# sevagh/xumx-sliCQ

Hardware: AMD Instinct MI355X
Metric: real-time factor (audio-s demixed / wall-s), 44.1 kHz stereo, offline model (higher is better)
Workload: dtype f32; 1 GPU; BASELINE configs[1]: offline model (Bark-262 sliCQT), one 240 s stereo track (10,584,000 samples, 5 chunks) per GPU, Wiener off (mix-phase), seeded synthetic weights; parallelism=one track per rank, 1 rank(s), no data-path collective

## Files before the change

### xumx_slicq_amd/csrc/plan.h

```cpp
#pragma once
#include <algorithm>
#include <map>
#include <mutex>
#include <tuple>
#include <vector>

#include <rocfft/rocfft.h>

#include "common.h"

namespace xsq {

struct FftPlan {
    rocfft_plan plan = nullptr;
    rocfft_execution_info info = nullptr;
    size_t work_bytes = 0;
};

struct TileTable {
    TileDev* d_tiles = nullptr;
    int ntiles = 0;
};

enum class TileKind { BandGemm, Dft4Full, CdaeGemm, CdaeSlab, CdaeWino, CdaeL1f, CdaeL4f };
struct TileKey {
    TileKind kind;
    int rows, S;
    int sub, flags;
    bool operator<(const TileKey& o) const {
        return std::tie(kind, rows, S, sub, flags) < std::tie(o.kind, o.rows, o.S, o.sub, o.flags);
    }
};

template <class D, class T>
static int upload(D*& dst, const T* src, size_t count) {
    dst = nullptr;
    if (!count) return XSQ_OK;
    XSQ_HIP(hipMalloc((void**)&dst, count * sizeof(T)));
    const hipError_t e = hipMemcpy(dst, src, count * sizeof(T), hipMemcpyHostToDevice);
    if (e != hipSuccess) { (void)hipFree(dst); dst = nullptr; }
    XSQ_HIP(e);
    return XSQ_OK;
}
template <class D, class T>
static int upload(D*& dst, const std::vector<T>& vec) { return upload(dst, vec.data(), vec.size()); }

template <class T, class Fill>
static int cached_tiles(std::mutex& mu, std::map<TileKey, TileTable>& cache, const TileKey& key, TileTable* out, Fill&& fill) {
    std::lock_guard<std::mutex> lk(mu);
    auto it = cache.find(key);
    if (it != cache.end()) { *out = it->second; return XSQ_OK; }
    std::vector<T> t;
    fill(t);
    TileTable tt;
    tt.ntiles = (int)t.size();
    if (int rc = upload(tt.d_tiles, t)) return rc;
    cache[key] = tt;
    *out = tt;
    return XSQ_OK;
}

template <class KeyFn>
static std::vector<int> order_descending(int n, KeyFn key) {
    std::vector<int> order(n);
    for (int i = 0; i < n; ++i) order[i] = i;
    std::stable_sort(order.begin(), order.end(), [&](int x, int y) { return key(x) > key(y); });
    return order;
}

struct BlockHost {
    int first_band, F, T;
    int64_t cum;
};

}

struct xsq_plan {
    int L = 0, tr = 0, h = 0, nbins = 0, nbands = 0, nblocks = 0;
    int64_t sumFT = 0;
    std::vector<xsq::BandDev> bands;
    std::vector<xsq::BlockHost> blocks;
    int band_radix4 = 1;
    void* d_bands4 = nullptr;
    float* d_pool4f = nullptr;
    float* d_pool4i = nullptr;
    int nbands4 = 0;
    std::vector<unsigned char> bands4_host;
    int64_t d4_max_block = 0;
    std::vector<int> bands4_m, bands4_small;
    int fft_backend = 0;
    float2* d_T = nullptr;
    unsigned short* d_tgt16 = nullptr;
    int* d_tgt = nullptr;
    int phase_begin[5] = {0, 0, 0, 0, 0};
    int packed_fft = 0;
    int short_inline = 0;
    void *d_s_item1 = nullptr, *d_s_tw1 = nullptr;
    int *d_s_item2 = nullptr, *d_s_tgt = nullptr;
    float* d_s_wd = nullptr;
    int short_n1 = 0, short_n2 = 0, short_nent = 0, short_sc0 = 0;
    int short_begin[5] = {0, 0, 0, 0, 0};
    int phase_long[4] = {0, 0, 0, 0};
    float* d_tw = nullptr;
    float* d_Wf = nullptr;
    float* d_Wi = nullptr;
    xsq::BandDev* d_bands = nullptr;
    int* d_cov_ptr = nullptr;
    int* d_cov_band = nullptr;
    std::mutex mu;
    std::map<std::pair<int, int>, xsq::FftPlan> fft;
    std::map<xsq::TileKey, xsq::TileTable> tiles;
};
```

### xumx_slicq_amd/csrc/slicqt.hip

```cpp
#include <algorithm>
#include <cmath>
#include <cstdarg>
#include <cstdio>
#include <cstdlib>
#include <cstring>

#include "../../include/xumx_slicq_hip.h"
#include "gemm_tile.h"
#include "plan.h"
#include "prof.h"
#include "slice_fft.h"
#include "band_dft4.h"
#include "band_dft4s.h"

namespace xsq {

static thread_local char g_err[1024] = "";
void set_error(const char* fmt, ...) {
    va_list ap;
    va_start(ap, fmt);
    vsnprintf(g_err, sizeof(g_err), fmt, ap);
    va_end(ap);
}

__global__ __launch_bounds__(256) void k_slice_window(const float* __restrict__ x,
                                                       const float* __restrict__ tw,
                                                       float* __restrict__ seg, int S, int64_t n, int L,
                                                       int h, const int64_t* __restrict__ xrows = nullptr,
                                                       const float* const* __restrict__ xslot = nullptr) {
    const int p = blockIdx.x * 256 + threadIdx.x;
    if (p >= L) return;
    const int row = blockIdx.y;
    const int bc = row / S, s = row - bc * S;
    const int64_t i = (int64_t)(2 * s - 2) * h + p;
    float v = 0.f;
    if (i >= 0 && i < n) v = tw[p] * (xslot ? *xslot : x)[(xrows ? xrows[bc] : (int64_t)bc * n) + i];
    seg[(int64_t)row * L + p] = v;
}

__global__ __launch_bounds__(256) void k_spectrum_gather(const float* __restrict__ Z,
                                                          const BandDev* __restrict__ bands,
                                                          const int* __restrict__ cov_ptr,
                                                          const int* __restrict__ cov_band,
                                                          float2* __restrict__ fr, int BC, int S, int nbins) {
    const int k = blockIdx.x * 256 + threadIdx.x;
    if (k >= nbins) return;
    const int row = blockIdx.y;
    const int bc = row / S, s = row - bc * S;
    const int64_t BCS = (int64_t)BC * S;
    float2 acc = make_float2(0.f, 0.f);
    for (int e = cov_ptr[k]; e < cov_ptr[k + 1]; ++e) {
        const BandDev b = bands[cov_band[e]];
        const int64_t off = 2 * (BCS * b.cum + (((int64_t)bc * b.F + b.f) * S + s) * b.Lg + (k - b.bin0));
        const float2 z = *reinterpret_cast<const float2*>(Z + off);
        acc.x += z.x;
        acc.y += z.y;
    }
    if (k == 0 || k == nbins - 1) acc.y = 0.f;
    fr[(int64_t)row * nbins + k] = acc;
}

__global__ __launch_bounds__(256) void k_overlap_add(const float* __restrict__ seg, float* __restrict__ y,
                                                      const int64_t* __restrict__ row_off,
                                                      int S, int64_t length, int L, int h) {
    const int64_t i = (int64_t)blockIdx.x * 256 + threadIdx.x;
    if (i >= length) return;
// ... 130 lines not shown
        if (mask) { v.x *= mk.x; v.y *= mk.x; v.z *= mk.y; v.w *= mk.y; }
        return v;
    }
    __device__ void epilogue(const Group& g, int row0, int n, const f32x16& a0, const f32x16& a1, bool wide) const {
        const bool c0 = n < g.N, c1 = wide && n + 32 < g.N;
#pragma unroll
        for (int r = 0; r < 16; ++r) {
            const int m = row0 + acc_row(r);
            if (m >= g.M) break;
            float* d = (row_len ? Z + 2 * ((int64_t)m * row_len + g.bin0) : Z + row_off(g, m)) + n;
            if (c0) d[0] = a0[r];
            if (c1) d[32] = a1[r];
        }
    }
};

constexpr int REMIX_MAX_BLOCKS = 256;
struct RemixArgs {
    const float* src;
    float* dst;
    int nch, R, S, cplx;
    float g[4][4];
    int use[4];
    int cum[REMIX_MAX_BLOCKS + 1];
};

__global__ __launch_bounds__(256) void k_remix_combine(RemixArgs a) {
#pragma clang fp contract(off)
    const int j = blockIdx.y, ch = blockIdx.z;
    const int64_t per = (int64_t)a.S * (a.cum[j + 1] - a.cum[j]) * a.cplx;
    const int64_t e = ((int64_t)blockIdx.x * 256 + threadIdx.x) * 4;
    if (e >= per) return;
    const int64_t base = (int64_t)a.S * a.cum[j] * a.cplx;
    const float* s = a.src + base * (4 * a.nch) + (int64_t)ch * per + e;
    float4 m[4];
#pragma unroll
    for (int t = 0; t < 4; ++t)
        m[t] = a.use[t] ? *reinterpret_cast<const float4*>(s + (int64_t)t * a.nch * per) : make_float4(0.f, 0.f, 0.f, 0.f);
    float* d = a.dst + base * ((int64_t)a.R * a.nch) + (int64_t)ch * per + e;
#pragma unroll
    for (int r = 0; r < 4; ++r) {
        if (r >= a.R) break;
        float4 acc = make_float4(0.f, 0.f, 0.f, 0.f);
#pragma unroll
        for (int t = 0; t < 4; ++t) {
            if (!a.use[t]) continue;
            const float g = a.g[r][t];
            acc.x = acc.x + g * m[t].x; acc.y = acc.y + g * m[t].y; acc.z = acc.z + g * m[t].z; acc.w = acc.w + g * m[t].w;
        }
        *reinterpret_cast<float4*>(d + (int64_t)r * a.nch * per) = acc;
    }
}

static int get_band_tiles(xsq_plan* P, int rows, TileTable* out) {
    const bool r4 = P->band_radix4 && P->nbands4 > 0;
    return cached_tiles<TileDev>(P->mu, P->tiles, TileKey{TileKind::BandGemm, rows, 0, 0, r4 ? 1 : 0}, out, [&](std::vector<TileDev>& t) {
        if (r4) {
            for (int i = (int)P->bands4_small.size() - 1; i >= 0; --i)
                push_group_tiles(t, P->bands4_small[i], rows, 2 * P->bands[P->bands4_small[i]].Lg);
        } else {
            for (int j = P->nbands - 1; j >= 0; --j) push_group_tiles(t, j, rows, 2 * P->bands[j].Lg);
        }
    });
}

#ifndef XSQ_D4_MIN_LG_DEFAULT
#define XSQ_D4_MIN_LG_DEFAULT 24
#endif

struct Switches {
    bool d4_sym = true;
    int d4_min_lg = XSQ_D4_MIN_LG_DEFAULT;
    Switches() {
        if (const char* e = getenv("XSQ_D4_SYM")) d4_sym = atoi(e) != 0;
        if (const char* e = getenv("XSQ_D4_MIN_LG")) d4_min_lg = atoi(e) >= 16 ? atoi(e) : d4_min_lg;
    }
};
static const Switches& switches() { static const Switches sw; return sw; }

static int get_dft4_full_tiles(xsq_plan* P, int rows, TileTable* out, int share, bool sym) {
    return cached_tiles<Tile4Dev>(P->mu, P->tiles, TileKey{TileKind::Dft4Full, rows, share, 0, sym ? 1 : 0}, out, [&](std::vector<Tile4Dev>& t) {
        const Band4Dev* b4 = reinterpret_cast<const Band4Dev*>(P->bands4_host.data());
        const int span = share > 0 ? share : rows, copies = share > 0 ? rows / share : 1;
        for (int i = P->nbands4 - 1; i >= 0; --i) {
            int ncb = (2 * P->bands4_m[i] + 15) / 16;
            if (sym) ncb = (P->bands4_m[i] / 2 + 1 + 15) / 16;
            for (int m0 = 0; m0 < span; m0 += D4H_ROWS)
                for (int k = 0; k < copies; ++k) t.push_back(Tile4Dev{m0 + k * span, ncb, b4[i]});
        }
    });
}

static int d4_ranges_ok(const xsq_plan* P, int64_t rows, const char* who) {
    if (!(P->band_radix4 && P->nbands4)) return XSQ_OK;
    XSQ_REQUIRE(8 * rows * P->d4_max_block < (1ll << 30) && (int64_t)8 * D4H_ROWS * std::max<int64_t>(P->nbins, P->sumFT) < (1ll << 30),
                "%s: %lld rows x %lld coefficients of a band block exceed 2^30 bytes; split the call (fewer stacked chunks)",
                who, (long long)rows, (long long)P->d4_max_block);
    return XSQ_OK;
}

template <bool FWD>
static int launch_dft4(xsq_plan* P, const Band4Args& a4, int rows, int share, hipStream_t stream) {
    const bool sym = switches().d4_sym;
    const bool masked = !FWD && a4.mask != nullptr;
    TileTable t;
    if (int rc = get_dft4_full_tiles(P, rows, &t, share, sym)) return rc;
    if (!t.ntiles) return XSQ_OK;
    auto kernel = masked ? band_dft4s_kernel<false, true> : band_dft4s_kernel<FWD, false>;
    if (!sym) kernel = masked ? band_dft4_full_kernel<false, 10, true> : band_dft4_full_kernel<FWD, 10, false>;
    hipLaunchKernelGGL(kernel, dim3(t.ntiles), dim3(sym ? 256 : D4H_NT), 0, stream, a4, (const Tile4Dev*)t.d_tiles, t.ntiles);
    return XSQ_OK;
}

static int get_fft(xsq_plan* P, int inverse, int batch, FftPlan* out) {
    std::lock_guard<std::mutex> lk(P->mu);
    auto key = std::make_pair(inverse, batch);
    auto it = P->fft.find(key);
    if (it != P->fft.end()) {
        *out = it->second;
        return XSQ_OK;
    }
    static std::once_flag once;
    std::call_once(once, [] { rocfft_setup(); });
    FftPlan f;
    size_t len = (size_t)P->L;
    rocfft_status st = rocfft_plan_create(&f.plan, rocfft_placement_notinplace,
                                          inverse ? rocfft_transform_type_real_inverse
                                                  : rocfft_transform_type_real_forward,
                                          rocfft_precision_single, 1, &len, (size_t)batch, nullptr);
    if (st != rocfft_status_success) {
        set_error("rocfft_plan_create(L=%d, batch=%d, inverse=%d) failed: %d", P->L, batch, inverse, (int)st);
        return XSQ_ERR_FFT;
    }
    rocfft_plan_get_work_buffer_size(f.plan, &f.work_bytes);
    if (rocfft_execution_info_create(&f.info) != rocfft_status_success) {
        set_error("rocfft_execution_info_create failed");
        return XSQ_ERR_FFT;
    }
    P->fft[key] = f;
    *out = f;
    return XSQ_OK;
}

static int run_fft(const FftPlan& f, void* in, void* out, void* work, hipStream_t stream) {
    if (rocfft_execution_info_set_stream(f.info, stream) != rocfft_status_success) {
        set_error("rocfft_execution_info_set_stream failed");
        return XSQ_ERR_FFT;
    }
    if (f.work_bytes) {
        if (rocfft_execution_info_set_work_buffer(f.info, work, f.work_bytes) != rocfft_status_success) {
            set_error("rocfft_execution_info_set_work_buffer failed");
            return XSQ_ERR_FFT;
        }
    }
    void* ib[1] = {in};
    void* ob[1] = {out};
    rocfft_status st = rocfft_execute(f.plan, ib, ob, f.info);
    if (st != rocfft_status_success) {
        set_error("rocfft_execute failed: %d", (int)st);
        return XSQ_ERR_FFT;
    }
    return XSQ_OK;
}
// ... 88 lines not shown
        }
    }
}

static void build_coverage(const xsq_plan* P, std::vector<int>& cov_ptr, std::vector<int>& cov_band) {
    cov_ptr.assign(P->nbins + 1, 0);
    std::vector<std::vector<int>> cov(P->nbins);
    for (int j = 0; j < P->nbands; ++j)
        for (int p = 0; p < P->bands[j].Lg; ++p) {
            const int k = P->bands[j].bin0 + p;
            if (k >= 0 && k <= P->L / 2) cov[k].push_back(j);
        }
    for (int k = 0; k < P->nbins; ++k) {
        cov_ptr[k + 1] = cov_ptr[k] + (int)cov[k].size();
        cov_band.insert(cov_band.end(), cov[k].begin(), cov[k].end());
    }
}

static bool build_slice_fft_tables(xsq_plan* P, std::vector<float2>& T, std::vector<int>& tgt, std::vector<unsigned short>& tgt16) {
    const int L = P->L, nbands = P->nbands;
    auto W = [&](int64_t j) {
        j %= L;
        return make_float2((float)std::cos(PI2 * j / L), (float)(-std::sin(PI2 * j / L)));
    };
    for (int k1 = 0; k1 < FFT_R1; ++k1)
        for (int m = 0; m < FFT_M1; ++m) T.push_back(W(2 * (int64_t)k1 * m));
    for (int k2 = 0; k2 < FFT_R2; ++k2)
        for (int n3 = 0; n3 < FFT_R3; ++n3) T.push_back(W(2 * (int64_t)FFT_R1 * n3 * k2));
    for (int k = 0; k <= FFT_N; ++k) T.push_back(W(k));
    bool ok = true;
    for (int ph = 0; ph < 4; ++ph) {
        P->phase_begin[ph] = (int)tgt.size();
        int last_end = -(1 << 30);
        for (int j = ph; j < nbands; j += 4) {
            BandDev& b = P->bands[j];
            b.ent = (int)tgt.size();
            const int lo = b.bin0 < 0 ? 0 : b.bin0;
            if (lo < last_end) ok = false;
            last_end = b.bin0 + b.Lg > L / 2 + 1 ? L / 2 + 1 : b.bin0 + b.Lg;
            for (int q = 0; q < b.Lg; ++q) {
                const int k = b.bin0 + q;
                tgt.push_back(k >= 0 && k <= L / 2 ? k : -1);
            }
        }
    }
    P->phase_begin[4] = (int)tgt.size();
    tgt16.assign(tgt.size() + 2, 0xFFFFu);
    for (size_t i = 0; i < tgt.size(); ++i) tgt16[i] = tgt[i] >= 0 ? (unsigned short)tgt[i] : 0xFFFFu;
    return ok;
}

static void build_radix4_tables(xsq_plan* P, const PlanArgs& A, std::vector<Band4Dev>& b4, std::vector<float>& pf, std::vector<float>& pi,
                                std::vector<char>& is_short) {
    const int d4_min_lg = switches().d4_min_lg;
    is_short.assign(A.nbands, 0);
    std::map<int, int64_t> doff, twoff, coff;
    auto alloc2 = [&](size_t n) { size_t o = pf.size(); pf.resize(o + n, 0.f); pi.resize(o + n, 0.f); return (int64_t)o; };
    for (int j = 0; j < A.nbands; ++j) {
        const BandDev& b = P->bands[j];
        if (b.Lg < d4_min_lg || b.Lg > 4 * D4_MPAD) { P->bands4_small.push_back(j); is_short[j] = 1; continue; }
        const int n = b.Lg, m = n / 4;
        Band4Dev d;
        memset(&d, 0, sizeof(d));
        d.Lg = n; d.m = m; d.bin0 = b.bin0; d.f = b.f; d.F = b.F; d.ent = b.ent; d.cum = b.cum; d.jband = j;
        d.ldd = (int)round_up(2 * m, 16);
        if (!doff.count(m)) {
            const int64_t o = alloc2((size_t)round_up(2 * m, 64) * d.ldd);
            doff[m] = o;
            for (int k = 0; k < m; ++k)
                for (int t1 = 0; t1 < m; ++t1) {
                    const int r = (int)(((int64_t)k * t1) % m);
                    const double cr = std::cos(PI2 * r / m), si = std::sin(PI2 * r / m);
                    for (int dir = 0; dir < 2; ++dir) {
                        std::vector<float>& pool = dir ? pi : pf;
                        const double dre = cr, dim = dir ? -si : si;
                        pool[o + (size_t)(2 * k) * d.ldd + 2 * t1] = (float)dre;
                        pool[o + (size_t)(2 * k) * d.ldd + 2 * t1 + 1] = (float)(-dim);
                        pool[o + (size_t)(2 * k + 1) * d.ldd + 2 * t1] = (float)dim;
                        pool[o + (size_t)(2 * k + 1) * d.ldd + 2 * t1 + 1] = (float)dre;
                    }
                }
        }
        d.d_off = doff[m];
        d.K2 = m / 2 + 1; d.ldc = (int)round_up(d.K2, 8);
        if (!coff.count(m)) {
            const size_t csz = (size_t)round_up(d.K2, 16) * d.ldc;
            const int64_t o = alloc2(2 * csz);
            coff[m] = o;
            for (int k = 0; k < d.K2; ++k)
                for (int nn = 0; nn < d.K2; ++nn) {
                    const int r = (int)(((int64_t)k * nn) % m);
                    const double cr = std::cos(PI2 * r / m), si = (nn == 0 || 2 * nn == m) ? 0.0 : std::sin(PI2 * r / m);
                    pf[o + (size_t)k * d.ldc + nn] = (float)cr;
                    pi[o + (size_t)k * d.ldc + nn] = (float)cr;
                    pf[o + csz + (size_t)k * d.ldc + nn] = (float)(-si);
                    pi[o + csz + (size_t)k * d.ldc + nn] = (float)si;
                }
        }
        d.c_off = coff[m];
        if (!twoff.count(n)) {
            const int mpad = (m + 7) & ~7;
            const int64_t o = alloc2((size_t)3 * mpad * 2);
            twoff[n] = o;
            for (int r = 1; r <= 3; ++r)
                for (int t1 = 0; t1 < m; ++t1) {
                    const int e = (r * t1) % n;
                    const double cr = std::cos(PI2 * e / n), si = std::sin(PI2 * e / n);
                    pf[o + 2 * ((size_t)(r - 1) * mpad + t1)] = (float)cr;
                    pf[o + 2 * ((size_t)(r - 1) * mpad + t1) + 1] = (float)si;
                    pi[o + 2 * ((size_t)(r - 1) * mpad + t1)] = (float)cr;
                    pi[o + 2 * ((size_t)(r - 1) * mpad + t1) + 1] = (float)(-si);
                }
        }
        d.tw_off = twoff[n];
        d.win_off = alloc2((size_t)round_up(n, 4));
        for (int q = 0; q < n; ++q) {
            pf[d.win_off + q] = (float)A.analysis_window(j, q);
            pi[d.win_off + q] = (float)A.synthesis_window(j, q);
        }
        b4.push_back(d);
        P->bands4_m.push_back(m);
        P->d4_max_block = std::max<int64_t>(P->d4_max_block, (int64_t)b.F * b.Lg);
    }
    P->nbands4 = (int)b4.size();
    P->bands4_host.assign(reinterpret_cast<const unsigned char*>(b4.data()),
                          reinterpret_cast<const unsigned char*>(b4.data()) + b4.size() * sizeof(Band4Dev));
}

struct ShortTables {
    std::vector<ShortItem1> item1;
    std::vector<float2> tw1;
    std::vector<int> codes, stgt;
    std::vector<float> swd;
    int nent = 0;
};
static bool build_short_schedule(xsq_plan* P, const PlanArgs& A, const std::vector<char>& is_short, ShortTables& H) {
    const int L = A.L, nbands = A.nbands;
    bool ok = true;
    int nent = 0, maxbin = 0;
    for (int j : P->bands4_small) {
        const BandDev& b = P->bands[j];
        if (b.Lg % 4 != 0 || b.Lg < 16 || b.Lg > 60) ok = false;
        nent += b.Lg;
        maxbin = std::max(maxbin, b.bin0 + b.Lg);
    }
    if (maxbin >= SHORT_SCRATCH0 || SHORT_SCRATCH0 + nent > FFT_N + 1) ok = false;
    if (!ok) return false;
    std::vector<std::pair<int, int>> item2;
    H.nent = nent;
    H.stgt.assign((size_t)nent, -1);
    H.swd.assign((size_t)nent, 0.f);
    int sc = 0;
    for (int ph = 0; ph < 4; ++ph) {
        P->short_begin[ph] = sc;
        for (int j : P->bands4_small) {
            if (j % 4 != ph) continue;
            const BandDev& b = P->bands[j];
            const int n = b.Lg, m = n / 4;
            for (int t1 = 0; t1 < m; ++t1) {
                H.item1.push_back(ShortItem1{(int)b.cum, b.F, b.f, n, t1, sc});
                for (int r = 1; r <= 3; ++r) {
                    const int e = (r * t1) % n;
                    H.tw1.push_back(make_float2((float)std::cos(PI2 * e / n), (float)(-std::sin(PI2 * e / n))));
                }
            }
            for (int r = 0; r < 4; ++r) {
                item2.push_back({m, ((sc + r * m) << 4) | m});
                for (int k = 0; k < m; ++k) {
                    const int q = 4 * k + r;
                    const int bin = b.bin0 + (q + n / 2) % n;
                    H.stgt[sc + r * m + k] = (bin >= 0 && bin <= L / 2) ? bin : -1;
                    H.swd[sc + r * m + k] = (float)A.synthesis_window(j, q);
                }
            }
            sc += n;
        }
// ... 5 lines not shown
        int lo = P->phase_begin[ph + 1];
        for (int j = ph; j < nbands; j += 4)
            if (!is_short[j]) { lo = P->bands[j].ent; break; }
        P->phase_long[ph] = lo;
        for (int j = ph; j < nbands; j += 4)
            if (is_short[j] && P->bands[j].ent >= lo) ok = false;
    }
    if (!(ok && H.item1.size() <= SHORT_MAX_BUTTERFLIES && H.codes.size() <= SHORT_MAX_DFTS && sc <= nent)) return false;
    for (int ph = 0; ph < 4; ++ph)
        if (P->short_begin[ph + 1] - P->short_begin[ph] > SHORT_MAX_PHASE_ENTRIES) return false;
    return true;
}

static int plan_build(xsq_plan* P, int L, int tr, int nbands, const int32_t* Lg, const int32_t* c,
                      const float* g, const double* gd, const float* tw) {
    PlanArgs A{L, tr, nbands, Lg, c, g, gd, tw, std::vector<int64_t>(nbands, 0)};
    for (int j = 1; j < nbands; ++j) A.g_off[j] = A.g_off[j - 1] + Lg[j - 1];
    int rc;
    if ((rc = build_band_tables(P, A))) return rc;

    std::vector<float> Wf, Wi;
    build_dense_matrices(P, A, Wf, Wi);
    if ((rc = upload(P->d_Wf, Wf))) return rc;
    if ((rc = upload(P->d_Wi, Wi))) return rc;

    std::vector<int> cov_ptr, cov_band;
    build_coverage(P, cov_ptr, cov_band);
    if ((rc = upload(P->d_cov_ptr, cov_ptr))) return rc;
    if ((rc = upload(P->d_cov_band, cov_band))) return rc;

    bool phase_table = false;
    if (L == FFT_L) {
        std::vector<float2> T;
        std::vector<int> tgt;
        std::vector<unsigned short> tgt16;
        phase_table = build_slice_fft_tables(P, T, tgt, tgt16);
        if ((rc = upload(P->d_T, T))) return rc;
        if (phase_table) {
            if ((rc = upload(P->d_tgt, tgt))) return rc;
            if ((rc = upload(P->d_tgt16, tgt16))) return rc;
        }
    }
    {
        std::vector<BandDev> dev = P->bands;
        if (!phase_table) for (BandDev& b : dev) b.ent = 0;
        if ((rc = upload(P->d_bands, dev))) return rc;
    }

    std::vector<char> is_short;
    {
        std::vector<Band4Dev> b4;
        std::vector<float> pf, pi;
        build_radix4_tables(P, A, b4, pf, pi, is_short);
        if (P->nbands4) {
            if ((rc = upload(P->d_bands4, b4))) return rc;
            if ((rc = upload(P->d_pool4f, pf))) return rc;
            if ((rc = upload(P->d_pool4i, pi))) return rc;
        }
    }
    if ((rc = upload(P->d_tw, tw, (size_t)L))) return rc;

    ShortTables H;
    if (P->d_tgt != nullptr && P->nbands4 > 0 && !P->bands4_small.empty() && build_short_schedule(P, A, is_short, H)) {
        if ((rc = upload(P->d_s_item1, H.item1))) return rc;
        if ((rc = upload(P->d_s_tw1, H.tw1))) return rc;
        if ((rc = upload(P->d_s_item2, H.codes))) return rc;
        if ((rc = upload(P->d_s_tgt, H.stgt))) return rc;
        if ((rc = upload(P->d_s_wd, H.swd))) return rc;
        P->short_n1 = (int)H.item1.size(); P->short_n2 = (int)H.codes.size();
        P->short_nent = H.nent; P->short_sc0 = SHORT_SCRATCH0;
    }
    return XSQ_OK;
}

}

using namespace xsq;

extern "C" {

int xsq_abi_version(void) { return XSQ_ABI_VERSION; }

#ifndef XSQ_BUILD_ARCH
#define XSQ_BUILD_ARCH "unknown"
#endif
#ifndef XSQ_BUILD_FLAGS
#define XSQ_BUILD_FLAGS ""
#endif
const char* xsq_build_info(void) { return "arch=" XSQ_BUILD_ARCH "; flags=" XSQ_BUILD_FLAGS "; date=" __DATE__ " " __TIME__; }
const char* xsq_last_error(void) { return g_err; }

int xsq_plan_create(xsq_plan** out, int L, int tr, int nbands, const int32_t* Lg, const int32_t* c,
                    const float* g, const double* gd, const float* tw) {
    XSQ_REQUIRE(out && Lg && c && g && gd && tw, "xsq_plan_create: null argument");
    XSQ_REQUIRE(L > 0 && L % 4 == 0 && tr % 2 == 0 && nbands >= 2, "xsq_plan_create: bad L/tr/nbands");
    xsq_plan* P = new xsq_plan();
    const int rc = plan_build(P, L, tr, nbands, Lg, c, g, gd, tw);
    if (rc != XSQ_OK) {
        xsq_plan_destroy(P);
        return rc;
    }
    *out = P;
    return XSQ_OK;
}

int xsq_plan_destroy(xsq_plan* P) {
    if (!P) return XSQ_OK;
// ... 93 lines not shown
}

int xsq_slicqt_forward_rows(xsq_plan* P, const float* x, const int64_t* x_rows, int BC, int64_t n, int64_t n_pad, float* coef,
                            float* xin, const float* mean, const float* scale, int split, void* ws, size_t ws_bytes,
                            void* stream_) {
    XSQ_REQUIRE(x, "xsq_slicqt_forward: null argument");
    return xsq_slicqt_forward_rows_indirect(P, x, nullptr, x_rows, BC, n, n_pad, coef, xin, mean, scale, split, ws, ws_bytes, stream_);
}

int xsq_slicqt_forward_rows_indirect(xsq_plan* P, const float* x, const float* const* x_slot, const int64_t* x_rows, int BC, int64_t n,
                                     int64_t n_pad, float* coef, float* xin, const float* mean, const float* scale, int split,
                                     void* ws, size_t ws_bytes, void* stream_) {
    XSQ_REQUIRE(P && (x || x_slot) && coef && ws, "xsq_slicqt_forward: null argument");
    XSQ_REQUIRE(!xin || (mean && scale), "xsq_slicqt_forward_xin: xin needs the mean / scale tables");
    XSQ_REQUIRE(BC > 0 && n > 0 && n_pad >= n, "xsq_slicqt_forward: BC=%d n=%lld n_pad=%lld", BC, (long long)n, (long long)n_pad);
    hipStream_t stream = (hipStream_t)stream_;
    const int S = xsq_plan_num_slices(P, n_pad);
    const int rows = BC * S;
    XSQ_REQUIRE(S >= 2, "xsq_slicqt_forward: signal too short");
    XSQ_REQUIRE((int64_t)BC * S <= 65535, "xsq_slicqt_forward: BC*S=%lld rows exceed one launch", (long long)BC * S);
    XSQ_REQUIRE((int64_t)2 * BC * S * (P->sumFT > P->nbins ? P->sumFT : P->nbins) < (1ll << 31),
                "xsq_slicqt_forward: BC*S=%lld rows exceed 2^31 floats of coefficients; split the call", (long long)BC * S);
    if (int rcg = d4_ranges_ok(P, (int64_t)BC * S, "xsq_slicqt_forward")) return rcg;
    FftPlan f;
    int rc = lds_fft(P) ? XSQ_OK : get_fft(P, 0, rows, &f);
    if (rc) return rc;
    char* w = (char*)ws;
    float* seg = (float*)w; w += al256((size_t)rows * P->L * 4);
    float* U = (float*)w;   w += al256((size_t)rows * P->nbins * 8);
    void* fwork = w;
    if ((size_t)(w - (char*)ws) + f.work_bytes > ws_bytes) {
        set_error("xsq_slicqt_forward: workspace too small (%zu needed, %zu given)",
                  (size_t)(w - (char*)ws) + f.work_bytes, ws_bytes);
        return XSQ_ERR_WORKSPACE;
    }
    if (lds_fft(P)) {
        XSQ_PROF("slice_rfft", stream);
        auto kernel = k_slice_rfft<512>;
#if XSQ_PACKED_FFT_KERNELS
        if (P->packed_fft) kernel = k_slice_rfft<512, true>;
#endif
        hipLaunchKernelGGL(kernel, dim3(rows), dim3(512), 0, stream, x, P->d_tw, fft_tables(P), (float2*)U, S, n, P->h, x_rows, x_slot);
    } else {
        { XSQ_PROF("slice_window", stream);
        hipLaunchKernelGGL(k_slice_window, dim3((P->L + 255) / 256, rows), dim3(256), 0, stream, x, P->d_tw, seg,
                           S, n, P->L, P->h, x_rows, x_slot); }
        { XSQ_PROF("rfft_L", stream); rc = run_fft(f, seg, U, fwork, stream); }
        if (rc) return rc;
    }
    TileTable tt;
    rc = get_band_tiles(P, rows, &tt);
    if (rc) return rc;
    BandFwdOp op{U, coef, P->d_bands, P->d_Wf, BC, S, P->nbins, P->L, xin, mean, scale, split};
    if (P->band_radix4 && P->nbands4) {
        Band4Args a4{(const Band4Dev*)P->d_bands4, P->d_pool4f, U, coef, BC, S, P->nbins, P->L, 0, nullptr, 0, xin, mean, scale, split};
        XSQ_PROF("band_analysis_dft4", stream);
        if ((rc = launch_dft4<true>(P, a4, rows, 0, stream))) return rc;
    }
    if (tt.ntiles) { XSQ_PROF("band_analysis_gemm", stream);
    hipLaunchKernelGGL((grouped_gemm_kernel<BandFwdOp>), dim3(tt.ntiles), dim3(256), 0, stream, op,
                       tt.d_tiles, tt.ntiles); }
    XSQ_HIP(hipGetLastError());
    return XSQ_OK;
}

size_t xsq_slicqt_inverse_workspace(xsq_plan* P, int BC, int S) {
    if (!P || BC <= 0 || S <= 0) return 0;
    const size_t rows = (size_t)BC * S;
    FftPlan f;
    if (!lds_fft(P) && get_fft(P, 1, (int)rows, &f)) return 0;
    if (lds_fft(P)) return al256(rows * P->sumFT * 8) + 256;
    return al256(rows * P->sumFT * 8) + al256(rows * P->nbins * 8) + al256(rows * P->L * 4) + al256(f.work_bytes) + 256;
}

int xsq_slicqt_inverse(xsq_plan* P, const float* coef, int BC, int S, int64_t length, float* y, void* ws,
                       size_t ws_bytes, void* stream_) {
    return xsq_slicqt_inverse_rows(P, coef, BC, S, length, y, nullptr, ws, ws_bytes, stream_);
}

static int inverse_impl(xsq_plan* P, const float* coef, const float* mask, int BCx, int BC, int S, int64_t length, float* y,
                        const int64_t* row_offsets, void* ws, size_t ws_bytes, void* stream_);

int xsq_slicqt_inverse_rows(xsq_plan* P, const float* coef, int BC, int S, int64_t length, float* y,
                            const int64_t* row_offsets, void* ws, size_t ws_bytes, void* stream_) {
    return inverse_impl(P, coef, nullptr, 0, BC, S, length, y, row_offsets, ws, ws_bytes, stream_);
}

int xsq_slicqt_inverse_masked(xsq_plan* P, const float* masks, const float* mix, int BC, int BCx, int S, int64_t length,
                              float* y, const int64_t* row_offsets, void* ws, size_t ws_bytes, void* stream_) {
    XSQ_REQUIRE(masks && mix, "xsq_slicqt_inverse_masked: null argument");
    XSQ_REQUIRE(BCx > 0 && BC % BCx == 0, "xsq_slicqt_inverse_masked: %d mix channels do not divide %d mask channels", BCx, BC);
    return inverse_impl(P, mix, masks, BCx, BC, S, length, y, row_offsets, ws, ws_bytes, stream_);
}

static int inverse_impl(xsq_plan* P, const float* coef, const float* mask, int BCx, int BC, int S, int64_t length, float* y,
                        const int64_t* row_offsets, void* ws, size_t ws_bytes, void* stream_) {
    XSQ_REQUIRE(P && coef && y && ws, "xsq_slicqt_inverse: null argument");
    XSQ_REQUIRE(BC > 0 && S >= 2 && length > 0, "xsq_slicqt_inverse: BC=%d S=%d length=%lld", BC, S,
                (long long)length);
    XSQ_REQUIRE(length <= (int64_t)2 * S * P->h, "xsq_slicqt_inverse: length %lld exceeds the %d slices",
                (long long)length, S);
    XSQ_REQUIRE((int64_t)BC * S <= 65535, "xsq_slicqt_inverse: BC*S=%lld rows exceed one launch", (long long)BC * S);
    XSQ_REQUIRE((int64_t)2 * BC * S * P->sumFT < (1ll << 31), "xsq_slicqt_inverse: the coefficient arena of BC*S=%lld rows "
                "exceeds 2^31 floats; split the call (fewer stacked chunks)", (long long)BC * S);
    if (int rcg = d4_ranges_ok(P, (int64_t)BC * S, "xsq_slicqt_inverse")) return rcg;
    hipStream_t stream = (hipStream_t)stream_;
    const int rows = BC * S;
    FftPlan f;
    int rc = lds_fft(P) ? XSQ_OK : get_fft(P, 1, rows, &f);
    if (rc) return rc;
    char* w = (char*)ws;
    float* Z = (float*)w;    w += al256((size_t)rows * P->sumFT * 8);
    float2* fr = (float2*)w; if (!lds_fft(P)) w += al256((size_t)rows * P->nbins * 8);
    float* seg = (float*)w;  if (!lds_fft(P)) w += al256((size_t)rows * P->L * 4);
    void* fwork = w;
    if ((size_t)(w - (char*)ws) + f.work_bytes > ws_bytes) {
        set_error("xsq_slicqt_inverse: workspace too small (%zu needed, %zu given)",
                  (size_t)(w - (char*)ws) + f.work_bytes, ws_bytes);
        return XSQ_ERR_WORKSPACE;
    }
    TileTable tt;
    rc = get_band_tiles(P, rows, &tt);
    if (rc) return rc;
    BandInvOp op{coef, Z, P->d_bands, P->d_Wi, BC, S, lds_fft(P) ? (int)P->sumFT : 0, mask, BCx};
    if (P->band_radix4 && P->nbands4) {
        Band4Args a4{(const Band4Dev*)P->d_bands4, P->d_pool4i, coef, Z, BC, S, P->nbins, P->L,
                     lds_fft(P) ? (int)P->sumFT : 0, mask, BCx, nullptr, nullptr, nullptr, 0};
        XSQ_PROF("band_synthesis_dft4", stream);
        if ((rc = launch_dft4<false>(P, a4, rows, mask ? BCx * S : 0, stream))) return rc;
    }
    const bool inl = lds_fft(P) && P->band_radix4 && P->short_inline && P->short_n1 > 0;
    if (tt.ntiles && !inl) { XSQ_PROF("band_synthesis_gemm", stream);
    hipLaunchKernelGGL((grouped_gemm_kernel<BandInvOp>), dim3(tt.ntiles), dim3(256), 0, stream, op,
                       tt.d_tiles, tt.ntiles); }
    if (lds_fft(P)) {
        XSQ_PROF("slice_irfft_ola", stream);
        GatherSched G;
        G.tgt = P->d_tgt; G.tgt16 = P->d_tgt16; G.row_len = (int)P->sumFT;
        for (int i = 0; i < 5; ++i) G.begin[i] = P->phase_begin[i];
        for (int i = 0; i < 4; ++i) G.lo[i] = inl ? P->phase_long[i] : P->phase_begin[i];
        ShortSched SS;
        memset(&SS, 0, sizeof(SS));
        if (inl) {
            SS.item1 = (const ShortItem1*)P->d_s_item1; SS.tw1 = (const float2*)P->d_s_tw1; SS.item2 = P->d_s_item2;
            SS.stgt = P->d_s_tgt; SS.swd = P->d_s_wd;
            SS.n1 = P->short_n1; SS.n2 = P->short_n2; SS.nent = P->short_nent; SS.sc0 = P->short_sc0;
            for (int i = 0; i < 5; ++i) SS.begin[i] = P->short_begin[i];
        }
        const ShortIn SI{coef, mask, BC, mask ? BCx : BC};
        bool fast4 = !inl && G.tgt16 != nullptr;
        for (int ph = 0; ph < 4; ++ph) fast4 = fast4 && (G.begin[ph + 1] - (G.lo[ph] & ~1) <= FAST4_MAX_PHASE_ENTRIES);
        auto kernel = inl ? k_slice_irfft<512, false, true> : fast4 ? k_slice_irfft<512, false, false, true> : k_slice_irfft<512>;
#if XSQ_PACKED_FFT_KERNELS
        if (P->packed_fft && !inl) kernel = fast4 ? k_slice_irfft<512, true, false, true> : k_slice_irfft<512, true>;
#endif
        for (int parity = 0; parity < 2; ++parity) {
            const int nsl = (S + 1 - parity) / 2;
            OlaArgs O{y, row_offsets, S, P->h, parity, length};
            hipLaunchKernelGGL(kernel, dim3(BC * nsl), dim3(512), 0, stream, (const float2*)Z, G, fft_tables(P), O, SS, SI);
        }
        XSQ_HIP(hipGetLastError());
        return XSQ_OK;
    } else {
        { XSQ_PROF("spectrum_gather", stream);
        hipLaunchKernelGGL(k_spectrum_gather, dim3((P->nbins + 255) / 256, rows), dim3(256), 0, stream, Z,
                           P->d_bands, P->d_cov_ptr, P->d_cov_band, fr, BC, S, P->nbins); }
        { XSQ_PROF("irfft_L", stream); rc = run_fft(f, fr, seg, fwork, stream); }
        if (rc) return rc;
    }
    { XSQ_PROF("overlap_add", stream);
    hipLaunchKernelGGL(k_overlap_add, dim3((unsigned)((length + 255) / 256), BC), dim3(256), 0, stream, seg, y,
                       row_offsets, S, length, P->L, P->h); }
    XSQ_HIP(hipGetLastError());
    return XSQ_OK;
}

static int remix_gains_ok(const float* gains, int R, const char* who) {
    XSQ_REQUIRE(gains, "%s: null gains", who);
    XSQ_REQUIRE(R >= 1 && R <= 4, "%s: R=%d mixes (1..4)", who, R);
    for (int i = 0; i < 4 * R; ++i) XSQ_REQUIRE(std::isfinite(gains[i]), "%s: gain [%d][%d] is not finite", who, i / 4, i % 4);
    return XSQ_OK;
}

size_t xsq_slicqt_remix_workspace(xsq_plan* P, int R, int B, int S, int wiener) {
    if (!P || R < 1 || R > 4 || B <= 0 || S <= 0) return 0;
    const size_t inv = xsq_slicqt_inverse_workspace(P, R * 2 * B, S);
    if (!inv) return 0;
// ... 40 lines not shown
```

Measured before the change: 55200 x real-time.

## Route short non-reflecting bands through a dedicated small radix-4 DFT kernel

Measured after the change: 55640 x real-time, median of 6. No clear change (+0.8%).

```diff
diff --git a/xumx_slicq_amd/csrc/band_route.h b/xumx_slicq_amd/csrc/band_route.h
--- /dev/null
+++ b/xumx_slicq_amd/csrc/band_route.h
@@ -0,0 +1,36 @@
+#pragma once
+#include <cstdlib>
+
+#ifndef XSQ_D4_MIN_LG_DEFAULT
+#error "XSQ_D4_MIN_LG_DEFAULT is defined in slicqt.hip, in front of this header"
+#endif
+
+namespace xsq {
+
+constexpr int XSQ_SMALL_MIN_LG = 16, XSQ_SMALL_MAX_LG = 56;
+constexpr int XSQ_R4_MAX_LG = 320;
+
+struct Switches {
+    bool d4_sym = true;
+    int d4_min_lg = XSQ_D4_MIN_LG_DEFAULT;
+    bool small_bands = true;
+    Switches() {
+        if (const char* e = getenv("XSQ_D4_SYM")) d4_sym = atoi(e) != 0;
+        if (const char* e = getenv("XSQ_D4_MIN_LG")) d4_min_lg = atoi(e) >= 16 ? atoi(e) : d4_min_lg;
+        if (const char* e = getenv("XSQ_SMALL_BANDS")) small_bands = atoi(e) != 0;
+    }
+};
+static const Switches& switches() { static const Switches sw; return sw; }
+
+enum class BandRoute { Dense = 0, Radix4 = 1, Small = 2 };
+
+static inline BandRoute band_route(int Lg, int bin0, int L, const Switches& sw) {
+    const bool reflect = bin0 < 0 || bin0 + Lg - 1 > L / 2;
+    const bool small_len = sw.small_bands && Lg % 4 == 0 && Lg >= XSQ_SMALL_MIN_LG && Lg <= XSQ_SMALL_MAX_LG;
+    if (small_len && !reflect) return BandRoute::Small;
+    if (Lg > XSQ_R4_MAX_LG) return BandRoute::Dense;
+    if (Lg >= sw.d4_min_lg || small_len) return BandRoute::Radix4;
+    return BandRoute::Dense;
+}
+
+}
diff --git a/xumx_slicq_amd/csrc/band_small.h b/xumx_slicq_amd/csrc/band_small.h
--- /dev/null
+++ b/xumx_slicq_amd/csrc/band_small.h
@@ -0,0 +1,172 @@
+#pragma once
+#include "band_dft4.h"
+
+namespace xsq {
+
+constexpr int SB_MIN_LG = 16, SB_MAX_LG = 56;
+constexpr int SB_MAX_K2 = SB_MAX_LG / 8 + 1;
+constexpr int SB_NT = 256, SB_MAX_ROWS = SB_NT / 3;
+constexpr int SB_TAB_LD = 8;
+static_assert(SB_MAX_K2 <= SB_TAB_LD, "the cos / sin table holds rows of 8 outputs");
+static inline int sb_tile_rows(int K2) { return SB_NT / K2; }
+
+template <bool FWD, bool MASKED = false>
+__global__ __launch_bounds__(SB_NT)
+void band_small_kernel(Band4Args a, const Tile4Dev* __restrict__ tiles, int ntiles) {
+#pragma clang fp contract(off)
+    static_assert(!(FWD && MASKED), "the mask product belongs to the synthesis");
+    __shared__ __attribute__((aligned(16))) float4 ab[SB_NT * 4 + SB_MAX_ROWS + 16];
+    __shared__ __attribute__((aligned(16))) float2 cs[SB_MAX_K2 * SB_TAB_LD];
+
+    const int tid = threadIdx.x;
+    const Tile4Dev t = tiles[xcd_remap(blockIdx.x, ntiles)];
+    const Band4Dev bd = t.bd;
+    const int nrows = t.ncb;
+    const int m_ = bd.m, Lg = bd.Lg, K2 = bd.K2, M = a.BC * a.S;
+    const int64_t BCS = (int64_t)a.BC * a.S;
+    const int mpad = (m_ + 7) & ~7;
+
+    const unsigned rcp = (65536u + (unsigned)K2 - 1u) / (unsigned)K2;
+    const int s_row = (int)(((unsigned)tid * rcp) >> 16), s_p = tid - s_row * K2;
+    const int row = t.m0 + s_row;
+    const bool row_ok = s_row < nrows && row < M;
+    const int rowc = row_ok ? row : 0;
+    const int bc = rowc / a.S, sl = rowc - bc * a.S;
+    const unsigned blk = (unsigned)(bd.F * Lg) * (unsigned)a.S;
+    const unsigned arow = (unsigned)(((bc * bd.F + bd.f) * a.S + sl) * Lg);
+
+    __amdgpu_buffer_rsrc_t rx, rm = buf_rsrc(a.src, 0);
+    unsigned vx, vm = BUF_OOB;
+    if (FWD) {
+        rx = buf_rsrc(a.src + 2 * ((int64_t)t.m0 * a.nbins), 8u * (unsigned)(nrows * a.nbins));
+        vx = row_ok ? 8u * (unsigned)(s_row * a.nbins + bd.bin0) : BUF_OOB;
+    } else if (!MASKED) {
+        rx = buf_rsrc(a.src + 2 * (BCS * bd.cum), 8u * a.BC * blk);
+        vx = row_ok ? 8u * arow : BUF_OOB;
+    } else {
+        rx = buf_rsrc(a.src + 2 * ((int64_t)a.BCx * a.S * bd.cum), 8u * a.BCx * blk);
+        rm = buf_rsrc(a.mask + BCS * bd.cum, 4u * a.BC * blk);
+        vx = row_ok ? 8u * (unsigned)((((bc % a.BCx) * bd.F + bd.f) * a.S + sl) * Lg) : BUF_OOB;
+        vm = row_ok ? 4u * arow : BUF_OOB;
+    }
+    const int n = s_p;
+    const bool own = n == 0 || 2 * n == m_;
+    const int t1a = n, t1b = own ? 0 : m_ - n;
+    float2 ra[4], rbq[4];
+    float ma[4], mb[4];
+    {
+        const unsigned oa = vx + 8u * (unsigned)t1a, ob = own ? BUF_OOB : vx + 8u * (unsigned)t1b;
+        const unsigned qa = vm + 4u * (unsigned)t1a, qb = own ? BUF_OOB : vm + 4u * (unsigned)t1b;
+#pragma unroll
+        for (int q4 = 0; q4 < 4; ++q4) {
+            const int qq = FWD ? ((q4 + 2) & 3) : q4;
+            ra[q4] = buf_ld2(rx, oa, 8 * qq * m_);
+            rbq[q4] = buf_ld2(rx, ob, 8 * qq * m_);
+            ma[q4] = 1.f; mb[q4] = 1.f;
+            if (MASKED) { ma[q4] = buf_ld1(rm, qa, 4 * q4 * m_); mb[q4] = buf_ld1(rm, qb, 4 * q4 * m_); }
+        }
+    }
+    const float2* const tw = reinterpret_cast<const float2*>(a.pool + bd.tw_off);
+    const float* const win = a.pool + bd.win_off;
+    if (tid < 8 * SB_MAX_K2) {
+        const int k = tid >> 3, nn = tid & 7;
+        if (k < K2 && nn < K2) {
+            const float* c = a.pool + bd.c_off + k * bd.ldc + nn;
+            cs[nn * SB_TAB_LD + k] = make_float2(c[0], c[((K2 + 15) & ~15) * bd.ldc]);
+        }
+    }
+    auto butterfly = [&](const float2 (&raw)[4], const float (&mk)[4], int t1, float2 (&y)[4]) {
+        float2 x[4];
+#pragma unroll
+        for (int q4 = 0; q4 < 4; ++q4) {
+            float2 v = raw[q4];
+            if (!FWD) {
+                if (MASKED) { v.x *= mk[q4]; v.y *= mk[q4]; }
+            } else {
+                const float g = win[t1 + q4 * m_];
+                v = make_float2(v.x * g, v.y * g);
+            }
+            x[q4] = v;
+        }
+        const float2 w1 = tw[t1], w2 = tw[mpad + t1], w3 = tw[2 * mpad + t1];
+        const float2 s0 = make_float2(x[0].x + x[2].x, x[0].y + x[2].y), s1 = make_float2(x[1].x + x[3].x, x[1].y + x[3].y);
+        const float2 d0 = make_float2(x[0].x - x[2].x, x[0].y - x[2].y), d1 = make_float2(x[1].x - x[3].x, x[1].y - x[3].y);
+        const float2 y2 = make_float2(s0.x - s1.x, s0.y - s1.y);
+        const float2 ym = make_float2(d0.x + d1.y, d0.y - d1.x);
+        const float2 yp = make_float2(d0.x - d1.y, d0.y + d1.x);
+        const float2 y1 = FWD ? yp : ym, y3 = FWD ? ym : yp;
+        y[0] = make_float2(s0.x + s1.x, s0.y + s1.y);
+        y[1] = make_float2(fmaf(y1.x, w1.x, -(y1.y * w1.y)), fmaf(y1.x, w1.y, y1.y * w1.x));
+        y[2] = make_float2(fmaf(y2.x, w2.x, -(y2.y * w2.y)), fmaf(y2.x, w2.y, y2.y * w2.x));
+        y[3] = make_float2(fmaf(y3.x, w3.x, -(y3.y * w3.y)), fmaf(y3.x, w3.y, y3.y * w3.x));
+    };
+    float4* const abrow = ab + s_row * (4 * K2 + 1);
+    {
+        float2 ya[4], yb[4];
+        butterfly(ra, ma, t1a, ya);
+        butterfly(rbq, mb, t1b, yb);
+        if (s_row < nrows)
+#pragma unroll
+            for (int r = 0; r < 4; ++r)
+                abrow[r * K2 + s_p] = make_float4(ya[r].x + yb[r].x, ya[r].y + yb[r].y, ya[r].x - yb[r].x, ya[r].y - yb[r].y);
+    }
+    const int k = s_p;
+    const bool mir_ok = k != 0 && 2 * k != m_;
+    const int q1 = 4 * k, q2 = mir_ok ? 4 * (m_ - k) : 0;
+    float4 w1 = make_float4(1.f, 1.f, 1.f, 1.f), w2 = w1;
+    float w_mu = 0.f, w_sc = 1.f;
+    if (!FWD) {
+        w1 = *reinterpret_cast<const float4*>(win + q1);
+        w2 = *reinterpret_cast<const float4*>(win + q2);
+    } else if (a.xin) { w_mu = a.mean[bd.jband]; w_sc = a.scale[bd.jband]; }
+    __syncthreads();
+
+    float pr[4], pi[4], qr[4], qi[4];
+#pragma unroll
+    for (int r = 0; r < 4; ++r) { pr[r] = 0.f; pi[r] = 0.f; qr[r] = 0.f; qi[r] = 0.f; }
+#pragma unroll
+    for (int nn = 0; nn < SB_MAX_K2; ++nn) {
+        if (nn >= K2) continue;
+        const float2 c = cs[nn * SB_TAB_LD + k];
+#pragma unroll
+        for (int r = 0; r < 4; ++r) {
+            const float4 v = abrow[r * K2 + nn];
+            pr[r] = fmaf(v.x, c.x, pr[r]); pi[r] = fmaf(v.y, c.x, pi[r]);
+            qr[r] = fmaf(v.z, c.y, qr[r]); qi[r] = fmaf(v.w, c.y, qi[r]);
+        }
+    }
+    const bool rowmajor = !FWD && a.row_len;
+    const float* const dbase = rowmajor ? a.dst + 2 * ((int64_t)t.m0 * a.row_len + bd.ent) : a.dst + 2 * (BCS * bd.cum);
+    const unsigned dbytes = rowmajor ? 8u * (unsigned)(nrows * a.row_len) : 8u * a.BC * blk;
+    const __amdgpu_buffer_rsrc_t rd = buf_rsrc(dbase, dbytes);
+    const __amdgpu_buffer_rsrc_t rxin = buf_rsrc(FWD && a.xin ? a.xin + BCS * bd.cum : a.dst, FWD && a.xin ? 4u * a.BC * blk : 0u);
+    const unsigned vrow = row_ok ? (rowmajor ? 8u * (unsigned)(s_row * a.row_len) : 8u * arow) : BUF_OOB;
+    const bool split = a.split;
+    const float wa[4] = {w1.x, w1.y, w1.z, w1.w}, wb[4] = {w2.x, w2.y, w2.z, w2.w};
+#pragma unroll
+    for (int rp = 0; rp < 2; ++rp) {
+        const int r0 = 2 * rp, r1 = r0 + 1;
+        float4 v1, v2;
+        v1.x = (pr[r0] + qi[r0]) * wa[r0]; v1.y = (pi[r0] - qr[r0]) * wa[r0];
+        v1.z = (pr[r1] + qi[r1]) * wa[r1]; v1.w = (pi[r1] - qr[r1]) * wa[r1];
+        v2.x = (pr[r0] - qi[r0]) * wb[r0]; v2.y = (pi[r0] + qr[r0]) * wb[r0];
+        v2.z = (pr[r1] - qi[r1]) * wb[r1]; v2.w = (pi[r1] + qr[r1]) * wb[r1];
+        unsigned p1 = 8u * (unsigned)(q1 + r0), p2 = 8u * (unsigned)(q2 + r0);
+        if (!FWD) {
+            p1 += 16u * (unsigned)m_; if (p1 >= 8u * (unsigned)Lg) p1 -= 8u * (unsigned)Lg;
+            p2 += 16u * (unsigned)m_; if (p2 >= 8u * (unsigned)Lg) p2 -= 8u * (unsigned)Lg;
+        }
+        const unsigned vo1 = vrow + p1, vo2 = vrow + (mir_ok ? p2 : BUF_OOB_COL);
+        buf_st4(v1, rd, vo1, 0);
+        buf_st4(v2, rd, vo2, 0);
+        if (FWD && a.xin) {
+            float2 u1 = make_float2(whiten_mag(v1.x, v1.y, w_mu, w_sc), whiten_mag(v1.z, v1.w, w_mu, w_sc));
+            float2 u2 = make_float2(whiten_mag(v2.x, v2.y, w_mu, w_sc), whiten_mag(v2.z, v2.w, w_mu, w_sc));
+            if (split) { bf3_words2(u1.x, u1.y, u1.x, u1.y); bf3_words2(u2.x, u2.y, u2.x, u2.y); }
+            buf_st2(u1, rxin, (vo1 >> 1) | (vo1 & (BUF_OOB | BUF_OOB_COL)), 0);
+            buf_st2(u2, rxin, (vo2 >> 1) | (vo2 & (BUF_OOB | BUF_OOB_COL)), 0);
+        }
+    }
+}
+
+}
diff --git a/xumx_slicq_amd/csrc/plan.h b/xumx_slicq_amd/csrc/plan.h
--- a/xumx_slicq_amd/csrc/plan.h
+++ b/xumx_slicq_amd/csrc/plan.h
@@ -22,7 +22,7 @@
     int ntiles = 0;
 };
 
-enum class TileKind { BandGemm, Dft4Full, CdaeGemm, CdaeSlab, CdaeWino, CdaeL1f, CdaeL4f };
+enum class TileKind { BandGemm, Dft4Full, BandSmall, CdaeGemm, CdaeSlab, CdaeWino, CdaeL1f, CdaeL4f };
 struct TileKey {
     TileKind kind;
     int rows, S;
@@ -88,6 +88,8 @@
     std::vector<unsigned char> bands4_host;
     int64_t d4_max_block = 0;
     std::vector<int> bands4_m, bands4_small;
+    int nbands4s = 0;
+    std::vector<unsigned char> bands4s_host;
     int fft_backend = 0;
     float2* d_T = nullptr;
     unsigned short* d_tgt16 = nullptr;
diff --git a/xumx_slicq_amd/csrc/slicqt.hip b/xumx_slicq_amd/csrc/slicqt.hip
--- a/xumx_slicq_amd/csrc/slicqt.hip
+++ b/xumx_slicq_amd/csrc/slicqt.hip
@@ -12,6 +12,17 @@
 #include "slice_fft.h"
 #include "band_dft4.h"
 #include "band_dft4s.h"
+#include "band_small.h"
+
+#ifndef XSQ_D4_MIN_LG_DEFAULT
+#define XSQ_D4_MIN_LG_DEFAULT 24
+#endif
+
+#include "band_route.h"
+namespace xsq {
+static_assert(XSQ_SMALL_MIN_LG == SB_MIN_LG && XSQ_SMALL_MAX_LG == SB_MAX_LG && XSQ_R4_MAX_LG == 4 * D4_MPAD,
+              "band_route.h quotes the limits of band_small.h and band_dft4.h");
+}
 
 namespace xsq {
 
@@ -248,8 +259,10 @@
     }
 }
 
+static inline bool r4_on(const xsq_plan* P) { return P->band_radix4 && (P->nbands4 > 0 || P->nbands4s > 0); }
+
 static int get_band_tiles(xsq_plan* P, int rows, TileTable* out) {
-    const bool r4 = P->band_radix4 && P->nbands4 > 0;
+    const bool r4 = r4_on(P);
     return cached_tiles<TileDev>(P->mu, P->tiles, TileKey{TileKind::BandGemm, rows, 0, 0, r4 ? 1 : 0}, out, [&](std::vector<TileDev>& t) {
         if (r4) {
             for (int i = (int)P->bands4_small.size() - 1; i >= 0; --i)
@@ -259,20 +272,6 @@
         }
     });
 }
-
-#ifndef XSQ_D4_MIN_LG_DEFAULT
-#define XSQ_D4_MIN_LG_DEFAULT 24
-#endif
-
-struct Switches {
-    bool d4_sym = true;
-    int d4_min_lg = XSQ_D4_MIN_LG_DEFAULT;
-    Switches() {
-        if (const char* e = getenv("XSQ_D4_SYM")) d4_sym = atoi(e) != 0;
-        if (const char* e = getenv("XSQ_D4_MIN_LG")) d4_min_lg = atoi(e) >= 16 ? atoi(e) : d4_min_lg;
-    }
-};
-static const Switches& switches() { static const Switches sw; return sw; }
 
 static int get_dft4_full_tiles(xsq_plan* P, int rows, TileTable* out, int share, bool sym) {
     return cached_tiles<Tile4Dev>(P->mu, P->tiles, TileKey{TileKind::Dft4Full, rows, share, 0, sym ? 1 : 0}, out, [&](std::vector<Tile4Dev>& t) {
@@ -288,8 +287,9 @@
 }
 
 static int d4_ranges_ok(const xsq_plan* P, int64_t rows, const char* who) {
-    if (!(P->band_radix4 && P->nbands4)) return XSQ_OK;
-    XSQ_REQUIRE(8 * rows * P->d4_max_block < (1ll << 30) && (int64_t)8 * D4H_ROWS * std::max<int64_t>(P->nbins, P->sumFT) < (1ll << 30),
+    if (!r4_on(P)) return XSQ_OK;
+    XSQ_REQUIRE(8 * rows * P->d4_max_block < (1ll << 30) &&
+                (int64_t)8 * std::max(D4H_ROWS, SB_MAX_ROWS) * std::max<int64_t>(P->nbins, P->sumFT) < (1ll << 30),
                 "%s: %lld rows x %lld coefficients of a band block exceed 2^30 bytes; split the call (fewer stacked chunks)",
                 who, (long long)rows, (long long)P->d4_max_block);
     return XSQ_OK;
@@ -305,6 +305,33 @@
     auto kernel = masked ? band_dft4s_kernel<false, true> : band_dft4s_kernel<FWD, false>;
     if (!sym) kernel = masked ? band_dft4_full_kernel<false, 10, true> : band_dft4_full_kernel<FWD, 10, false>;
     hipLaunchKernelGGL(kernel, dim3(t.ntiles), dim3(sym ? 256 : D4H_NT), 0, stream, a4, (const Tile4Dev*)t.d_tiles, t.ntiles);
+    return XSQ_OK;
+}
+
+static int get_small_tiles(xsq_plan* P, int rows, TileTable* out, int share) {
+    return cached_tiles<Tile4Dev>(P->mu, P->tiles, TileKey{TileKind::BandSmall, rows, share, 0, 0}, out, [&](std::vector<Tile4Dev>& t) {
+        const Band4Dev* b = reinterpret_cast<const Band4Dev*>(P->bands4s_host.data());
+        const int span = share > 0 ? share : rows, copies = share > 0 ? rows / share : 1;
+        for (int i = 0; i < P->nbands4s;) {
+            int e = i + 1;
+            while (e < P->nbands4s && e < i + 4 && b[e].K2 == b[i].K2) ++e;
+            const int rt = sb_tile_rows(b[i].K2);
+            for (int m0 = 0; m0 < span; m0 += rt)
+                for (int g = i; g < e; ++g)
+                    for (int k = 0; k < copies; ++k) t.push_back(Tile4Dev{m0 + k * span, std::min(rt, span - m0), b[g]});
+            i = e;
+        }
+    });
+}
+
+template <bool FWD>
+static int launch_small(xsq_plan* P, const Band4Args& a4, int rows, int share, hipStream_t stream) {
+    const bool masked = !FWD && a4.mask != nullptr;
+    TileTable t;
+    if (int rc = get_small_tiles(P, rows, &t, share)) return rc;
+    if (!t.ntiles) return XSQ_OK;
+    auto kernel = masked ? band_small_kernel<false, true> : band_small_kernel<FWD, false>;
+    hipLaunchKernelGGL(kernel, dim3(t.ntiles), dim3(SB_NT), 0, stream, a4, (const Tile4Dev*)t.d_tiles, t.ntiles);
     return XSQ_OK;
 }
 
@@ -499,19 +526,21 @@
 
 static void build_radix4_tables(xsq_plan* P, const PlanArgs& A, std::vector<Band4Dev>& b4, std::vector<float>& pf, std::vector<float>& pi,
                                 std::vector<char>& is_short) {
-    const int d4_min_lg = switches().d4_min_lg;
+    std::vector<Band4Dev> b4s;
     is_short.assign(A.nbands, 0);
     std::map<int, int64_t> doff, twoff, coff;
     auto alloc2 = [&](size_t n) { size_t o = pf.size(); pf.resize(o + n, 0.f); pi.resize(o + n, 0.f); return (int64_t)o; };
     for (int j = 0; j < A.nbands; ++j) {
         const BandDev& b = P->bands[j];
-        if (b.Lg < d4_min_lg || b.Lg > 4 * D4_MPAD) { P->bands4_small.push_back(j); is_short[j] = 1; continue; }
+        const BandRoute route = band_route(b.Lg, b.bin0, A.L, switches());
+        if (route == BandRoute::Dense) { P->bands4_small.push_back(j); is_short[j] = 1; continue; }
+        const bool small = route == BandRoute::Small;
         const int n = b.Lg, m = n / 4;
         Band4Dev d;
         memset(&d, 0, sizeof(d));
         d.Lg = n; d.m = m; d.bin0 = b.bin0; d.f = b.f; d.F = b.F; d.ent = b.ent; d.cum = b.cum; d.jband = j;
         d.ldd = (int)round_up(2 * m, 16);
-        if (!doff.count(m)) {
+        if (!small && !doff.count(m)) {
             const int64_t o = alloc2((size_t)round_up(2 * m, 64) * d.ldd);
             doff[m] = o;
             for (int k = 0; k < m; ++k)
@@ -528,7 +557,7 @@
                     }
                 }
         }
-        d.d_off = doff[m];
+        d.d_off = small ? 0 : doff[m];
         d.K2 = m / 2 + 1; d.ldc = (int)round_up(d.K2, 8);
         if (!coff.count(m)) {
             const size_t csz = (size_t)round_up(d.K2, 16) * d.ldc;
@@ -565,10 +594,15 @@
             pf[d.win_off + q] = (float)A.analysis_window(j, q);
             pi[d.win_off + q] = (float)A.synthesis_window(j, q);
         }
+        P->d4_max_block = std::max<int64_t>(P->d4_max_block, (int64_t)b.F * b.Lg);
+        if (small) { b4s.push_back(d); continue; }
         b4.push_back(d);
         P->bands4_m.push_back(m);
-        P->d4_max_block = std::max<int64_t>(P->d4_max_block, (int64_t)b.F * b.Lg);
-    }
+    }
+    std::stable_sort(b4s.begin(), b4s.end(), [](const Band4Dev& x, const Band4Dev& y) { return x.ent < y.ent; });
+    P->nbands4s = (int)b4s.size();
+    P->bands4s_host.assign(reinterpret_cast<const unsigned char*>(b4s.data()),
+                           reinterpret_cast<const unsigned char*>(b4s.data()) + b4s.size() * sizeof(Band4Dev));
     P->nbands4 = (int)b4.size();
     P->bands4_host.assign(reinterpret_cast<const unsigned char*>(b4.data()),
                           reinterpret_cast<const unsigned char*>(b4.data()) + b4.size() * sizeof(Band4Dev));
@@ -680,7 +714,7 @@
         std::vector<Band4Dev> b4;
         std::vector<float> pf, pi;
         build_radix4_tables(P, A, b4, pf, pi, is_short);
-        if (P->nbands4) {
+        if (P->nbands4 || P->nbands4s) {
             if ((rc = upload(P->d_bands4, b4))) return rc;
             if ((rc = upload(P->d_pool4f, pf))) return rc;
             if ((rc = upload(P->d_pool4i, pi))) return rc;
@@ -880,14 +914,15 @@
     rc = get_band_tiles(P, rows, &tt);
     if (rc) return rc;
     BandFwdOp op{U, coef, P->d_bands, P->d_Wf, BC, S, P->nbins, P->L, xin, mean, scale, split};
-    if (P->band_radix4 && P->nbands4) {
-        Band4Args a4{(const Band4Dev*)P->d_bands4, P->d_pool4f, U, coef, BC, S, P->nbins, P->L, 0, nullptr, 0, xin, mean, scale, split};
+    const Band4Args a4{(const Band4Dev*)P->d_bands4, P->d_pool4f, U, coef, BC, S, P->nbins, P->L, 0, nullptr, 0, xin, mean, scale, split};
+    if (r4_on(P) && P->nbands4) {
         XSQ_PROF("band_analysis_dft4", stream);
         if ((rc = launch_dft4<true>(P, a4, rows, 0, stream))) return rc;
     }
-    if (tt.ntiles) { XSQ_PROF("band_analysis_gemm", stream);
-    hipLaunchKernelGGL((grouped_gemm_kernel<BandFwdOp>), dim3(tt.ntiles), dim3(256), 0, stream, op,
-                       tt.d_tiles, tt.ntiles); }
+    if ((r4_on(P) && P->nbands4s) || tt.ntiles) { XSQ_PROF("band_analysis_gemm", stream);
+    if (r4_on(P) && (rc = launch_small<true>(P, a4, rows, 0, stream))) return rc;
+    if (tt.ntiles) hipLaunchKernelGGL((grouped_gemm_kernel<BandFwdOp>), dim3(tt.ntiles), dim3(256), 0, stream, op,
+                                      tt.d_tiles, tt.ntiles); }
     XSQ_HIP(hipGetLastError());
     return XSQ_OK;
 }
@@ -951,16 +986,18 @@
     rc = get_band_tiles(P, rows, &tt);
     if (rc) return rc;
     BandInvOp op{coef, Z, P->d_bands, P->d_Wi, BC, S, lds_fft(P) ? (int)P->sumFT : 0, mask, BCx};
-    if (P->band_radix4 && P->nbands4) {
-        Band4Args a4{(const Band4Dev*)P->d_bands4, P->d_pool4i, coef, Z, BC, S, P->nbins, P->L,
-                     lds_fft(P) ? (int)P->sumFT : 0, mask, BCx, nullptr, nullptr, nullptr, 0};
+    const Band4Args a4{(const Band4Dev*)P->d_bands4, P->d_pool4i, coef, Z, BC, S, P->nbins, P->L,
+                       lds_fft(P) ? (int)P->sumFT : 0, mask, BCx, nullptr, nullptr, nullptr, 0};
+    if (r4_on(P) && P->nbands4) {
         XSQ_PROF("band_synthesis_dft4", stream);
         if ((rc = launch_dft4<false>(P, a4, rows, mask ? BCx * S : 0, stream))) return rc;
     }
     const bool inl = lds_fft(P) && P->band_radix4 && P->short_inline && P->short_n1 > 0;
-    if (tt.ntiles && !inl) { XSQ_PROF("band_synthesis_gemm", stream);
-    hipLaunchKernelGGL((grouped_gemm_kernel<BandInvOp>), dim3(tt.ntiles), dim3(256), 0, stream, op,
-                       tt.d_tiles, tt.ntiles); }
+    const bool dense = tt.ntiles && !inl;
+    if ((r4_on(P) && P->nbands4s) || dense) { XSQ_PROF("band_synthesis_gemm", stream);
+    if (r4_on(P) && (rc = launch_small<false>(P, a4, rows, mask ? BCx * S : 0, stream))) return rc;
+    if (dense) hipLaunchKernelGGL((grouped_gemm_kernel<BandInvOp>), dim3(tt.ntiles), dim3(256), 0, stream, op,
+                                  tt.d_tiles, tt.ntiles); }
     if (lds_fft(P)) {
         XSQ_PROF("slice_irfft_ola", stream);
         GatherSched G;
```
